# lslrh/DynaMask

Hardware: AMD Instinct MI355X
Metric: img/s (DynaMask mask-head path, 512 RoIs/img, fixed 28x28 exit; ms_per_step = ms per RoI batch) (higher is better)
Workload: dtype f32

## Files before the change

### dynamask_amd/csrc/deform_conv.hip

```cpp
#include "common.h"

namespace {

struct DcnArgs {
  const float* x;
  const float* offset;
  int NB, C, H, W, HW, Q;
  const float* wp;
  int Cout, CoutP, KQ, dg, relu;
  int q_begin = 0;
  float* out;
  int MT;
  float* ws = nullptr;
  long long ws_stride = 0, ws_floats = 0;
  int ksplit = 1, kchan = 0;
  const float* w2t = nullptr;
  const float* b2 = nullptr;
  float* out2 = nullptr;
  int M2 = 0, w2_ld = 0, out2_ct = 0, store_out = 1;
};

typedef float dm_f32x2 __attribute__((ext_vector_type(2)));

__device__ __forceinline__ float dcn_bilinear(float wt0, float wt1, float wb0, float wb1, float ta, float tb, float ba, float bb) {
  return __builtin_fmaf(wb1, bb, __builtin_fmaf(wb0, ba, __builtin_fmaf(wt1, tb, wt0 * ta)));
}

template <int WGM, int WGN, int WM, int WN>
__global__ __launch_bounds__(WGM* WGN * 64) void deform_conv_kernel(DcnArgs a) {
  constexpr int CK = 8;
  constexpr int TM = WGM * WM * 32;
  constexpr int TN = WGN * WN * 32;
  constexpr int NT = WGM * WGN * 64;
  constexpr int TG = NT / TN;
  constexpr int MAXT = (9 + TG - 1) / TG;
  constexpr int A_F4 = 9 * 2 * TM;
  constexpr int A_PER_T = (A_F4 + NT - 1) / NT;
  static_assert(NT % TN == 0, "threads must tile the pixel columns");

  extern __shared__ __attribute__((aligned(16))) float lds[];
  const int kc_begin = (a.ksplit > 1) ? (int)blockIdx.y * a.kchan : 0;
  const int kc_end = (a.ksplit > 1) ? min(a.C, kc_begin + a.kchan) : a.C;
  float* const e_out = (a.ksplit > 1) ? a.ws + (size_t)blockIdx.y * a.ws_stride : a.out;
  const int e_relu = (a.ksplit > 1) ? 0 : a.relu;
  dm_f32x4* ldsA = reinterpret_cast<dm_f32x4*>(lds);
  dm_f32x4* ldsB = reinterpret_cast<dm_f32x4*>(lds) + A_F4;

  const int tid = threadIdx.x;
  const int lane = tid & 63, wave = tid >> 6;
  const int wave_m = wave / WGN, wave_n = wave % WGN;
  const int hi = lane >> 5, l31 = lane & 31;
  int m_tile, n_tile;
  {
    const int b = blockIdx.x, grp = 8 * a.MT;
    const int full = (gridDim.x / grp) * grp;
    if (b < full) {
      const int g = b / grp, r = b - g * grp;
      m_tile = r / 8;
      n_tile = g * 8 + (r & 7);
    } else {
      const int r = b - full;
      m_tile = r % a.MT;
      n_tile = full / a.MT + r / a.MT;
    }
  }
  const int m0 = m_tile * TM;
  const int q0 = a.q_begin + n_tile * TN;
  const int HW = a.HW, W = a.W, H = a.H;

  int col_n[WN], col_p[WN];
  bool col_ok[WN];
#pragma unroll
  for (int wn = 0; wn < WN; ++wn) {
    int q = q0 + (wave_n * WN + wn) * 32 + l31;
    col_ok[wn] = q < a.Q;
    q = min(q, a.Q - 1);
    col_n[wn] = q / HW;
    col_p[wn] = q - col_n[wn] * HW;
  }

  const int gj = tid % TN;
  const int tg = tid / TN;
  int gq = q0 + gj;
  const bool g_ok = gq < a.Q;
  gq = min(gq, a.Q - 1);
  const int gn = gq / HW;
  const int gp = gq - gn * HW;
  const int gy = gp / W, gx = gp - gy * W;

  int ot[MAXT], ob[MAXT];
  float wt0[MAXT], wt1[MAXT], wb0[MAXT], wb1[MAXT];
  int cur_group = -1;
  const int cpg = a.C / a.dg;

  auto load_params = [&](int group) {
    const float* offp = a.offset + ((size_t)gn * a.dg + group) * 18 * HW + gp;
#pragma unroll
    for (int t = 0; t < MAXT; ++t) {
      const int tap = tg + t * TG;
      ot[t] = ob[t] = 0;
      wt0[t] = wt1[t] = wb0[t] = wb1[t] = 0.f;
      if (tap < 9 && g_ok) {
        const int ki = tap / 3, kj = tap - ki * 3;
        const float off_h = offp[(size_t)(2 * tap) * HW];
        const float off_w = offp[(size_t)(2 * tap + 1) * HW];
        const float h_im = (float)(gy - 1 + ki) + off_h;
        const float w_im = (float)(gx - 1 + kj) + off_w;
        if (h_im > -1.f && w_im > -1.f && h_im < (float)H && w_im < (float)W) {
          const int h_low = (int)floorf(h_im), w_low = (int)floorf(w_im);
          const float lh = h_im - (float)h_low, lw = w_im - (float)w_low;
          const float hh = 1.f - lh, hw = 1.f - lw;
          const float wr_t = (h_low >= 0) ? hh : 0.f;
          const float wr_b = (h_low + 1 <= H - 1) ? lh : 0.f;
          const int rt = min(max(h_low, 0), H - 1), rbm = min(max(h_low + 1, 0), H - 1);
          const int cb = min(max(w_low, 0), W - 2);
          const float wc0 = (cb == w_low ? hw : 0.f) + (cb == w_low + 1 ? lw : 0.f);
          const float wc1 = (cb + 1 == w_low ? hw : 0.f) + (cb + 1 == w_low + 1 ? lw : 0.f);
          ot[t] = rt * W + cb;
          ob[t] = rbm * W + cb;
          wt0[t] = wr_t * wc0; wt1[t] = wr_t * wc1;
          wb0[t] = wr_b * wc0; wb1[t] = wr_b * wc1;
        }
      }
    }
  };

  dm_f32x16 acc[WM][WN];
#pragma unroll
  for (int i = 0; i < WM; ++i)
#pragma unroll
    for (int j = 0; j < WN; ++j)
#pragma unroll
      for (int r = 0; r < 16; ++r) acc[i][j][r] = 0.f;

  struct __attribute__((packed, aligned(4))) F2 { float a, b; };
  dm_f32x4 ra[A_PER_T];
  dm_f32x4 raw[MAXT * 4];
  dm_f32x4 rb0[MAXT];

  auto prefetch_a = [&](int c0) {
#pragma unroll
    for (int i = 0; i < A_PER_T; ++i) {
      const int idx = tid + i * NT;
      dm_f32x4 v = {0.f, 0.f, 0.f, 0.f};
      if (idx < A_F4) {
        const int m = idx % TM;
        const int tq = idx / TM;
        const int qd = tq & 1;
        const int tap = tq >> 1;
        if (m0 + m < a.CoutP)
          v = *reinterpret_cast<const dm_f32x4*>(a.wp + (((size_t)tap * a.KQ + (c0 >> 2) + qd) * a.CoutP + m0 + m) * 4);
      }
      ra[i] = v;
    }
  };
  auto issue_quad = [&](int c0, int qd) {
    const float* xp = a.x + ((size_t)gn * a.C + c0 + qd * 4) * HW;
#pragma unroll
    for (int t = 0; t < MAXT; ++t) {
#pragma unroll
      for (int e = 0; e < 4; ++e) {
        const float* xc = xp + (size_t)e * HW;
        const F2 top = *reinterpret_cast<const F2*>(xc + ot[t]);
        const F2 bot = *reinterpret_cast<const F2*>(xc + ob[t]);
        dm_f32x4 v = {top.a, top.b, bot.a, bot.b};
        raw[t * 4 + e] = v;
      }
    }
  };
  auto combine = [&](int t) {
    dm_f32x4 v;
#pragma unroll
    for (int e = 0; e < 4; ++e) {
      const dm_f32x4 l = raw[t * 4 + e];
      v[e] = dcn_bilinear(wt0[t], wt1[t], wb0[t], wb1[t], l[0], l[1], l[2], l[3]);
// ... 211 lines not shown
    for (int i = 0; i < A_PER_T; ++i) {
      const int idx = tid + i * NT;
      const int m = idx % TM, tq = idx / TM;
      const int mm = min(m0 + m, a.CoutP - 1);
      ra[i] = *reinterpret_cast<const dm_f32x4*>(a.wp + (((size_t)(3 * g + (tq >> 1)) * a.KQ + (c0 >> 2) + (tq & 1)) * a.CoutP + mm) * 4);
    }
  };
  auto store_a = [&](int slot) {
#pragma unroll
    for (int i = 0; i < A_PER_T; ++i) ldsA[slot * AS_F4 + tid + i * NT] = ra[i];
  };
  auto load_x = [&](int c0) {
    const float* xc = a.x + ((size_t)n0 * a.C + c0) * HW;
#pragma unroll
    for (int i = 0; i < X_PER_T; ++i) {
#pragma unroll
      for (int e = 0; e < 4; ++e) rx[i][e] = xc[x_off[i] + e * HW];
    }
  };
  auto store_x = [&](int buf) {
#pragma unroll
    for (int i = 0; i < X_PER_T; ++i) {
      const int idx = tid + i * NT;
      if (idx < 4 * HW) ldsX[buf * xbuf + idx] = rx[i];
    }
  };
  auto gather3 = [&](int t0, int slot, int buf) {
    const dm_f32x4* xq = ldsX + buf * xbuf + xbase;
#pragma unroll
    for (int u = 0; u < 3; ++u) {
      const int tap = t0 + u;
      const dm_f32x4* pt = xq + (otb[tap] & 0xffff);
      const dm_f32x4* pb = xq + (otb[tap] >> 16);
      const dm_f32x4 tl = pt[0], tr = pt[1], bl = pb[0], br = pb[1];
      dm_f32x4 v;
#pragma unroll
      for (int e = 0; e < 4; ++e) v[e] = dcn_bilinear(wt0[tap], wt1[tap], wb0[tap], wb1[tap], tl[e], tr[e], bl[e], br[e]);
      ldsB[slot * BS_F4 + (u * 2 + gh) * TN + gj] = v;
    }
  };
  auto step = [&](int slot, bool fill, int t0, int gbuf) {
    const dm_f32x4* xq = ldsX + gbuf * xbuf + xbase;
#pragma unroll
    for (int u = 0; u < 3; ++u) {
      dm_f32x4 av[2], bv[2];
#pragma unroll
      for (int i = 0; i < 2; ++i) av[i] = ldsA[slot * AS_F4 + (u * 2 + hi) * TM + (wave_m * 2 + i) * 32 + l31];
#pragma unroll
      for (int j = 0; j < 2; ++j) bv[j] = ldsB[slot * BS_F4 + (u * 2 + hi) * TN + (wave_n * 2 + j) * 32 + l31];
      const int tap = t0 + u;
      dm_f32x4 tl, tr, bl, br;
      if (fill) {
        const dm_f32x4* pt = xq + (otb[tap] & 0xffff);
        const dm_f32x4* pb = xq + (otb[tap] >> 16);
        tl = pt[0]; tr = pt[1]; bl = pb[0]; br = pb[1];
      }
      __builtin_amdgcn_sched_barrier(0);
#pragma unroll
      for (int e = 0; e < 2; ++e)
#pragma unroll
        for (int i = 0; i < 2; ++i)
#pragma unroll
          for (int j = 0; j < 2; ++j) acc[i][j] = __builtin_amdgcn_mfma_f32_32x32x2f32(av[i][e], bv[j][e], acc[i][j], 0, 0, 0);
      __builtin_amdgcn_sched_barrier(0);
      if (fill) {
        dm_f32x4 v;
#pragma unroll
        for (int e = 0; e < 4; ++e) v[e] = dcn_bilinear(wt0[tap], wt1[tap], wb0[tap], wb1[tap], tl[e], tr[e], bl[e], br[e]);
        ldsB[(slot ^ 1) * BS_F4 + (u * 2 + gh) * TN + gj] = v;
      }
      __builtin_amdgcn_sched_barrier(0);
#pragma unroll
      for (int e = 2; e < 4; ++e)
#pragma unroll
        for (int i = 0; i < 2; ++i)
#pragma unroll
          for (int j = 0; j < 2; ++j) acc[i][j] = __builtin_amdgcn_mfma_f32_32x32x2f32(av[i][e], bv[j][e], acc[i][j], 0, 0, 0);
      __builtin_amdgcn_sched_barrier(0);
    }
  };

  int cur_group = kc_begin / cpg;
  load_params(cur_group);
  load_x(kc_begin);
  load_a(kc_begin, 0);
  store_x(0);
  store_a(0);
  load_a(kc_begin, 1);
  __syncthreads();
  gather3(0, 0, 0);
  __syncthreads();
  int slot = 0;
  for (int c0 = kc_begin, buf = 0; c0 < kc_end; c0 += 8, buf ^= 1) {
    const int cn = c0 + 8;
    const bool more = cn < kc_end;
    if (more) load_x(cn);
    store_a(slot ^ 1);
    load_a(c0, 2);
    step(slot, true, 3, buf);
    __syncthreads();
    slot ^= 1;
    store_a(slot ^ 1);
    if (more) {
      load_a(cn, 0);
      store_x(buf ^ 1);
    }
    step(slot, true, 6, buf);
    __syncthreads();
    slot ^= 1;
    if (more) {
      const int group = cn / cpg;
      if (group != cur_group) {
        cur_group = group;
        load_params(group);
      }
      store_a(slot ^ 1);
      load_a(cn, 1);
    }
    step(slot, more, 0, buf ^ 1);
    __syncthreads();
    slot ^= 1;
  }

  {
    float* pj[2];
#pragma unroll
    for (int j = 0; j < 2; ++j) pj[j] = e_out + (size_t)col_n[j] * a.Cout * HW + col_p[j];
    const int co_lane = m0 + wave_m * 64 + 4 * hi;
    const size_t off_lane = (size_t)co_lane * HW;
    const bool relu = e_relu != 0;
#pragma unroll
    for (int i = 0; i < 2; ++i)
#pragma unroll
      for (int r = 0; r < 16; ++r) {
        const int k = i * 32 + (r & 3) + 8 * (r >> 2);
        if (co_lane + k < a.Cout) {
          const size_t o = off_lane + (size_t)k * HW;
#pragma unroll
          for (int j = 0; j < 2; ++j)
            if (col_ok[j]) {
              float v = acc[i][j][r];
              if (relu) v = fmaxf(v, 0.f);
              pj[j][o] = v;
            }
        }
      }
  }
}

__global__ __launch_bounds__(256, 2) void deform_conv_c256_kernel(DcnArgs a) {
  constexpr int TN = 64, NT = 256;
  constexpr int BS_F4 = 3 * 2 * TN;
  constexpr int X_PER_T = 4;
  extern __shared__ __attribute__((aligned(16))) float lds[];
  dm_f32x4* ldsB = reinterpret_cast<dm_f32x4*>(lds);
  dm_f32x4* ldsX = ldsB + 2 * BS_F4;

  const int tid = threadIdx.x, lane = tid & 63, wave = tid >> 6;
  const int hi = lane >> 5, l31 = lane & 31;
  const int q0 = a.q_begin + (int)blockIdx.x * TN;
  const int HW = a.HW, W = a.W, H = a.H;
  const int n0 = q0 / HW;
  const int xbuf = 2 * 2 * HW;

  const int gj = tid & 63, gh = (tid >> 6) & 1, rb = tid >> 7;
  int gq = q0 + gj;
  const bool g_ok = gq < a.Q;
  gq = min(gq, a.Q - 1);
  const int gn = gq / HW, gp = gq - gn * HW;
  const int gy = gp / W, gx = gp - gy * W;
  const int xbase = ((gn - n0) * 2 + gh) * HW;

  int otb[3][2];
  float wt0[3][2], wt1[3][2], wb0[3][2], wb1[3][2];
  const int cpg = a.C / a.dg;
  auto load_params = [&](int group) {
    const float* offp = a.offset + ((size_t)gn * a.dg + group) * 18 * HW + gp;
#pragma unroll
    for (int s = 0; s < 3; ++s)
#pragma unroll
      for (int r = 0; r < 2; ++r) {
        otb[s][r] = 0;
        wt0[s][r] = wt1[s][r] = wb0[s][r] = wb1[s][r] = 0.f;
        if (g_ok) {
          const int ki = s, kj = r ? 2 : rb, tap = 3 * s + kj;
          const float h_im = (float)(gy - 1 + ki) + offp[(size_t)(2 * tap) * HW];
          const float w_im = (float)(gx - 1 + kj) + offp[(size_t)(2 * tap + 1) * HW];
          if (h_im > -1.f && w_im > -1.f && h_im < (float)H && w_im < (float)W) {
            const int h_low = (int)floorf(h_im), w_low = (int)floorf(w_im);
            const float lh = h_im - (float)h_low, lw = w_im - (float)w_low;
            const float hh = 1.f - lh, hw = 1.f - lw;
            const float wr_t = (h_low >= 0) ? hh : 0.f;
            const float wr_b = (h_low + 1 <= H - 1) ? lh : 0.f;
            const int rt = min(max(h_low, 0), H - 1), rbm = min(max(h_low + 1, 0), H - 1);
            const int cb = min(max(w_low, 0), W - 2);
            const float wc0 = (cb == w_low ? hw : 0.f) + (cb == w_low + 1 ? lw : 0.f);
            const float wc1 = (cb + 1 == w_low ? hw : 0.f) + (cb + 1 == w_low + 1 ? lw : 0.f);
            otb[s][r] = (rt * W + cb) | ((rbm * W + cb) << 16);
            wt0[s][r] = wr_t * wc0; wt1[s][r] = wr_t * wc1;
            wb0[s][r] = wr_b * wc0; wb1[s][r] = wr_b * wc1;
          }
        }
      }
  };

  dm_f32x16 acc[2][2];
#pragma unroll
  for (int i = 0; i < 2; ++i)
#pragma unroll
    for (int j = 0; j < 2; ++j)
#pragma unroll
      for (int r = 0; r < 16; ++r) acc[i][j][r] = 0.f;

  dm_f32x4 rx[X_PER_T];
  const __amdgpu_buffer_rsrc_t xsrc = __builtin_amdgcn_make_buffer_rsrc(
      const_cast<float*>(a.x) + (size_t)n0 * a.C * HW, 0, min(2, a.NB - n0) * a.C * HW * 4, 0x00020000);
  const __amdgpu_buffer_rsrc_t wsrc = __builtin_amdgcn_make_buffer_rsrc(const_cast<float*>(a.wp), 0, 9 * a.KQ * a.CoutP * 16, 0x00020000);
  unsigned x_off[X_PER_T];
#pragma unroll
  for (int i = 0; i < X_PER_T; ++i) {
    const int idx = tid + i * NT;
    const int img = idx / (2 * HW), r = idx - img * 2 * HW;
    const int quad = r / HW, px = r - quad * HW;
    const int ii = (idx < 4 * HW) ? img : 0, qq = (idx < 4 * HW) ? quad : 0, pp = (idx < 4 * HW) ? px : 0;
    x_off[i] = 4u * (unsigned)(((min(n0 + ii, a.NB - 1) - n0) * a.C + qq * 4) * HW + pp);
  }
  unsigned a_off[2];
#pragma unroll
  for (int i = 0; i < 2; ++i) a_off[i] = 16u * (unsigned)(hi * a.CoutP + min(wave * 64 + i * 32 + l31, a.CoutP - 1));
  const int a_quad = a.CoutP * 16, a_tap = a.KQ * a_quad;
  auto load_a1 = [&](dm_f32x4 (&dst)[6], int c0, int g, int u) {
    const int so = (3 * g + u) * a_tap + (c0 >> 2) * a_quad;
#pragma unroll
    for (int i = 0; i < 2; ++i) dst[u * 2 + i] = __builtin_bit_cast(dm_f32x4, __builtin_amdgcn_raw_buffer_load_b128(wsrc, a_off[i], so, 0));
  };
  auto load_x = [&](int c0) {
#pragma unroll
    for (int e = 0; e < 4; ++e) {
      const int so = (c0 + e) * HW * 4;
#pragma unroll
      for (int i = 0; i < X_PER_T; ++i) rx[i][e] = __builtin_bit_cast(float, __builtin_amdgcn_raw_buffer_load_b32(xsrc, x_off[i], so, 0));
    }
  };
  auto store_x = [&](int buf) {
#pragma unroll
    for (int i = 0; i < X_PER_T; ++i) {
      const int idx = tid + i * NT;
      if (idx < 4 * HW) ldsX[buf * xbuf + idx] = rx[i];
    }
  };
  auto whole_read = [&](const dm_f32x4* xq, int s, dm_f32x4& tl, dm_f32x4& tr, dm_f32x4& bl, dm_f32x4& br) {
    const dm_f32x4* pt = xq + (otb[s][0] & 0xffff);
    const dm_f32x4* pb = xq + (otb[s][0] >> 16);
    tl = pt[0]; tr = pt[1]; bl = pb[0]; br = pb[1];
  };
  auto whole_write = [&](int slot, int s, const dm_f32x4& tl, const dm_f32x4& tr, const dm_f32x4& bl, const dm_f32x4& br) {
    dm_f32x4 v;
#pragma unroll
    for (int e = 0; e < 4; ++e) v[e] = dcn_bilinear(wt0[s][0], wt1[s][0], wb0[s][0], wb1[s][0], tl[e], tr[e], bl[e], br[e]);
    ldsB[slot * BS_F4 + (rb * 2 + gh) * TN + gj] = v;
  };
  auto half_read = [&](const dm_f32x4* xq, int s, dm_f32x2& tl, dm_f32x2& tr, dm_f32x2& bl, dm_f32x2& br) {
    const dm_f32x2* pt = reinterpret_cast<const dm_f32x2*>(xq + (otb[s][1] & 0xffff)) + rb;
    const dm_f32x2* pb = reinterpret_cast<const dm_f32x2*>(xq + (otb[s][1] >> 16)) + rb;
    tl = pt[0]; tr = pt[2]; bl = pb[0]; br = pb[2];
  };
  auto half_write = [&](int slot, int s, const dm_f32x2& tl, const dm_f32x2& tr, const dm_f32x2& bl, const dm_f32x2& br) {
    dm_f32x2 v;
#pragma unroll
    for (int e = 0; e < 2; ++e) v[e] = dcn_bilinear(wt0[s][1], wt1[s][1], wb0[s][1], wb1[s][1], tl[e], tr[e], bl[e], br[e]);
    reinterpret_cast<dm_f32x2*>(&ldsB[slot * BS_F4 + (2 * 2 + gh) * TN + gj])[rb] = v;
  };
  auto step = [&](const dm_f32x4 (&cur)[6], dm_f32x4 (&nxt)[6], int slot, bool fill, int sn, int gbuf, bool pre, int pc0, int pg) {
    const dm_f32x4* xq = ldsX + gbuf * xbuf + xbase;
#pragma unroll
    for (int u = 0; u < 3; ++u) {
      dm_f32x4 bv[2];
#pragma unroll
      for (int j = 0; j < 2; ++j) bv[j] = ldsB[slot * BS_F4 + (u * 2 + hi) * TN + j * 32 + l31];
      dm_f32x4 tl, tr, bl, br;
      dm_f32x2 htl, htr, hbl, hbr;
      if (fill && u == 0) whole_read(xq, sn, tl, tr, bl, br);
      if (fill && u == 1) half_read(xq, sn, htl, htr, hbl, hbr);
      if (pre) load_a1(nxt, pc0, pg, u);
      __builtin_amdgcn_sched_barrier(0);
#pragma unroll
      for (int e = 0; e < 2; ++e)
#pragma unroll
        for (int i = 0; i < 2; ++i)
#pragma unroll
          for (int j = 0; j < 2; ++j) acc[i][j] = __builtin_amdgcn_mfma_f32_32x32x2f32(cur[u * 2 + i][e], bv[j][e], acc[i][j], 0, 0, 0);
      __builtin_amdgcn_sched_barrier(0);
      if (fill && u == 0) whole_write(slot ^ 1, sn, tl, tr, bl, br);
      if (fill && u == 1) half_write(slot ^ 1, sn, htl, htr, hbl, hbr);
      __builtin_amdgcn_sched_barrier(0);
#pragma unroll
      for (int e = 2; e < 4; ++e)
#pragma unroll
        for (int i = 0; i < 2; ++i)
#pragma unroll
          for (int j = 0; j < 2; ++j) acc[i][j] = __builtin_amdgcn_mfma_f32_32x32x2f32(cur[u * 2 + i][e], bv[j][e], acc[i][j], 0, 0, 0);
      __builtin_amdgcn_sched_barrier(0);
    }
  };
  int cur_group = 0;
  auto chunk = [&](dm_f32x4 (&p)[6], dm_f32x4 (&q)[6], int c0, int buf, int slot) {
    const int cn = c0 + 8;
    const bool more = cn < a.C;
    if (more) load_x(cn);
    step(p, q, slot, true, 1, buf, true, c0, 1);
    __syncthreads();
    if (more) store_x(buf ^ 1);
    step(q, p, slot ^ 1, true, 2, buf, true, c0, 2);
    __syncthreads();
    if (more) {
      const int group = cn / cpg;
      if (group != cur_group) {
        cur_group = group;
        load_params(group);
      }
    }
    step(p, q, slot, more, 0, buf ^ 1, more, cn, 0);
    __syncthreads();
  };

  dm_f32x4 a0[6], a1[6];
  load_params(0);
  load_x(0);
#pragma unroll
  for (int u = 0; u < 3; ++u) load_a1(a0, 0, 0, u);
  store_x(0);
  __syncthreads();
  {
    const dm_f32x4* xq = ldsX + xbase;
    dm_f32x4 tl, tr, bl, br;
    dm_f32x2 htl, htr, hbl, hbr;
    whole_read(xq, 0, tl, tr, bl, br);
    half_read(xq, 0, htl, htr, hbl, hbr);
    whole_write(0, 0, tl, tr, bl, br);
    half_write(0, 0, htl, htr, hbl, hbr);
  }
  __syncthreads();
  for (int c0 = 0; c0 < a.C; c0 += 16) {
    chunk(a0, a1, c0, 0, 0);
    if (c0 + 8 < a.C) chunk(a1, a0, c0 + 8, 1, 1);
  }

  {
    float* pj[2];
    bool col_ok[2];
#pragma unroll
    for (int j = 0; j < 2; ++j) {
      int q = q0 + j * 32 + l31;
      col_ok[j] = q < a.Q;
      q = min(q, a.Q - 1);
      const int n = q / HW;
      pj[j] = a.out + (size_t)n * a.Cout * HW + (q - n * HW);
    }
    const int co_lane = wave * 64 + 4 * hi;
    const size_t off_lane = (size_t)co_lane * HW;
    const bool relu = a.relu != 0;
#pragma unroll
    for (int i = 0; i < 2; ++i)
#pragma unroll
      for (int r = 0; r < 16; ++r) {
        const int k = i * 32 + (r & 3) + 8 * (r >> 2);
        if (co_lane + k < a.Cout) {
          const size_t o = off_lane + (size_t)k * HW;
#pragma unroll
          for (int j = 0; j < 2; ++j)
            if (col_ok[j]) {
              float v = acc[i][j][r];
              if (relu) v = fmaxf(v, 0.f);
              pj[j][o] = v;
            }
        }
      }
  }
}

constexpr int DCN_NEAR_ROWS = 5;

template <int WM, int WGM, int XR>
__global__ __launch_bounds__(256, 2) void deform_conv_band_kernel(DcnArgs a, int tiles_per_img, int BR) {
  constexpr int TM = WM * WGM * 32, TN = (4 / WGM) * 32, NT = 256;
  constexpr int A_F4 = 9 * 2 * TM;
  constexpr int A_PER_T = (A_F4 + NT - 1) / NT;
  extern __shared__ __attribute__((aligned(16))) float lds[];
  const int kc_begin = (a.ksplit > 1) ? (int)blockIdx.y * a.kchan : 0;
  const int kc_end = (a.ksplit > 1) ? min(a.C, kc_begin + a.kchan) : a.C;
  float* const e_out = (a.ksplit > 1) ? a.ws + (size_t)blockIdx.y * a.ws_stride : a.out;
  const int e_relu = (a.ksplit > 1) ? 0 : a.relu;
  dm_f32x4* ldsA = reinterpret_cast<dm_f32x4*>(lds);
  dm_f32x4* ldsX = reinterpret_cast<dm_f32x4*>(lds) + A_F4;
  const int tid = threadIdx.x, lane = tid & 63, wave = tid >> 6;
  const int hi = lane >> 5, l31 = lane & 31;
  const int wave_m = wave % WGM, wave_n = wave / WGM;
  const int HW = a.HW, W = a.W, H = a.H;
  const int PS = BR * W, PS4 = PS >> 2;
  const int n = blockIdx.x / tiles_per_img, tile = blockIdx.x - n * tiles_per_img;
  const int p0 = tile * TN;
  const int p_end = min(p0 + TN, HW);
  const int y_first = p0 / W, y_last = (p_end - 1) / W;
  const int band_y0 = min(max(y_first - (BR - (y_last - y_first + 1)) / 2, 0), H - BR);
  int gp = p0 + wave_n * 32 + l31;
  const bool g_ok = gp < HW;
  gp = min(gp, HW - 1);
  const int gy = gp / W, gx = gp - gy * W;

  int otb[9];
  float wt0[9], wt1[9], wb0[9], wb1[9];
  unsigned oob = 0, any_oob = 0;
  const int cpg = a.C / a.dg;
  auto load_params = [&](int group) {
    const float* offp = a.offset + ((size_t)n * a.dg + group) * 18 * HW + gp;
    oob = 0;
#pragma unroll
    for (int tap = 0; tap < 9; ++tap) {
      otb[tap] = 0;
      wt0[tap] = wt1[tap] = wb0[tap] = wb1[tap] = 0.f;
      if (g_ok) {
        const int ki = tap / 3, kj = tap - ki * 3;
        const float h_im = (float)(gy - 1 + ki) + offp[(size_t)(2 * tap) * HW];
        const float w_im = (float)(gx - 1 + kj) + offp[(size_t)(2 * tap + 1) * HW];
        if (h_im > -1.f && w_im > -1.f && h_im < (float)H && w_im < (float)W) {
          const int h_low = (int)floorf(h_im), w_low = (int)floorf(w_im);
          const float lh = h_im - (float)h_low, lw = w_im - (float)w_low;
          const float hh = 1.f - lh, hw = 1.f - lw;
          const float wr_t = (h_low >= 0) ? hh : 0.f;
          const float wr_b = (h_low + 1 <= H - 1) ? lh : 0.f;
          const int rt = min(max(h_low, 0), H - 1), rbm = min(max(h_low + 1, 0), H - 1);
          const int cb = min(max(w_low, 0), W - 2);
          const float wc0 = (cb == w_low ? hw : 0.f) + (cb == w_low + 1 ? lw : 0.f);
          const float wc1 = (cb + 1 == w_low ? hw : 0.f) + (cb + 1 == w_low + 1 ? lw : 0.f);
          if (rt >= gy - DCN_NEAR_ROWS && rbm <= gy + DCN_NEAR_ROWS) {
            otb[tap] = ((rt - band_y0) * W + cb) | (((rbm - band_y0) * W + cb) << 16);
            wt0[tap] = wr_t * wc0; wt1[tap] = wr_t * wc1;
            wb0[tap] = wr_b * wc0; wb1[tap] = wr_b * wc1;
          } else {
            oob |= 1u << tap;
          }
        }
      }
    }
    any_oob = 0;
#pragma unroll
    for (int tap = 0; tap < 9; ++tap)
      if (__ballot((oob >> tap) & 1u) != 0ull) any_oob |= 1u << tap;
  };

  dm_f32x16 acc[WM];
#pragma unroll
  for (int i = 0; i < WM; ++i)
#pragma unroll
    for (int r = 0; r < 16; ++r) acc[i][r] = 0.f;

  dm_f32x4 ra[A_PER_T], rx[XR];
  unsigned a_off[A_PER_T];
#pragma unroll
  for (int i = 0; i < A_PER_T; ++i) {
    const int idx = min(tid + i * NT, A_F4 - 1);
    const int m = idx % TM, tq = idx / TM;
    a_off[i] = (unsigned)((((size_t)(tq >> 1) * a.KQ + (tq & 1)) * a.CoutP + min(m, a.CoutP - 1)) * 4);
  }
  auto load_a = [&](int c0) {
    const float* wb = a.wp + (size_t)(c0 >> 2) * a.CoutP * 4;
#pragma unroll
    for (int i = 0; i < A_PER_T; ++i) ra[i] = *reinterpret_cast<const dm_f32x4*>(wb + a_off[i]);
  };
  auto load_x = [&](int c0) {
    const float* xb = a.x + ((size_t)n * a.C + c0) * HW + (size_t)band_y0 * W;
#pragma unroll
    for (int i = 0; i < XR; ++i) {
      const int idx = tid + i * NT;
      const int off = (idx < PS) ? idx : (idx < 2 * PS ? 4 * HW + idx - PS : 0);
#pragma unroll
      for (int e = 0; e < 4; ++e) rx[i][e] = xb[off + e * HW];
    }
  };
  auto store_ax = [&]() {
#pragma unroll
    for (int i = 0; i < A_PER_T; ++i) {
      const int idx = tid + i * NT;
      if (idx < A_F4) ldsA[idx] = ra[i];
    }
#pragma unroll
    for (int i = 0; i < XR; ++i) {
      const int idx = tid + i * NT;
      if (idx < 2 * PS) ldsX[idx] = rx[i];
    }
  };
  struct __attribute__((packed, aligned(4))) F2 { float a, b; };

  int cur_group = kc_begin / cpg;
  load_params(cur_group);
  load_a(kc_begin);
  load_x(kc_begin);
  for (int c0 = kc_begin; c0 < kc_end; c0 += 8) {
// ... 95 lines not shown
    {
      const dm_f32x4* src = reinterpret_cast<const dm_f32x4*>(a.w2t);
      dm_f32x4* dst = reinterpret_cast<dm_f32x4*>(lds);
      for (int idx = tid; idx < a.Cout * (ld2 / 4); idx += NT) dst[idx] = src[idx];
    }
    __syncthreads();
    const float* w2t = lds;
    dm_f32x16 acc2[MT2];
#pragma unroll
    for (int t = 0; t < MT2; ++t)
#pragma unroll
      for (int r = 0; r < 16; ++r) acc2[t][r] = 0.f;
#pragma unroll
    for (int i = 0; i < WM; ++i)
#pragma unroll
      for (int r = 0; r < 16; ++r) {
        const int kb = i * 32 + (r & 3) + 8 * (r >> 2) + 4 * hi;
        const float b = fmaxf(acc[i][r], 0.f);
#pragma unroll
        for (int t = 0; t < MT2; ++t)
          if (t * 32 < ld2) acc2[t] = __builtin_amdgcn_mfma_f32_32x32x2f32(w2t[kb * ld2 + t * 32 + l31], b, acc2[t], 0, 0, 0);
      }
    const int p = p0 + wave_n * 32 + l31;
    if (p < HW) {
      float* po2 = a.out2 + (size_t)n * a.out2_ct * HW + p;
#pragma unroll
      for (int t = 0; t < MT2; ++t)
#pragma unroll
        for (int r = 0; r < 16; ++r) {
          const int co = t * 32 + (r & 3) + 8 * (r >> 2) + 4 * hi;
          if (co < a.M2) po2[(size_t)co * HW] = fmaxf(acc2[t][r] + a.b2[co], 0.f);
        }
    }
    if (!a.store_out) return;
  }
  {
    const int p = p0 + wave_n * 32 + l31;
    if (p < HW) {
      float* po = e_out + (size_t)n * a.Cout * HW + p;
      const bool relu = e_relu != 0;
#pragma unroll
      for (int i = 0; i < WM; ++i)
#pragma unroll
        for (int r = 0; r < 16; ++r) {
          const int co = (wave_m * WM + i) * 32 + (r & 3) + 8 * (r >> 2) + 4 * hi;
          if (co < a.Cout) {
            float v = acc[i][r];
            if (relu) v = fmaxf(v, 0.f);
            po[(size_t)co * HW] = v;
          }
        }
    }
  }
}

__global__ __launch_bounds__(256) void dcn_splitk_reduce_kernel(const float* __restrict__ ws, int splits, long long stride,
                                                               long long total, int relu, float* __restrict__ out) {
  const bool v4 = splits > 0;
  splits = v4 ? splits : -splits;
  if (v4) {
    const float4* ws4 = reinterpret_cast<const float4*>(ws);
    float4* out4 = reinterpret_cast<float4*>(out);
    const long long total4 = total >> 2, stride4 = stride >> 2;
    for (long long e = (long long)blockIdx.x * blockDim.x + threadIdx.x; e < total4; e += (long long)gridDim.x * blockDim.x) {
      float4 v = ws4[e];
      for (int s_ = 1; s_ < splits; ++s_) {
        const float4 w = ws4[(size_t)s_ * stride4 + e];
        v.x += w.x; v.y += w.y; v.z += w.z; v.w += w.w;
      }
      if (relu) { v.x = fmaxf(v.x, 0.f); v.y = fmaxf(v.y, 0.f); v.z = fmaxf(v.z, 0.f); v.w = fmaxf(v.w, 0.f); }
      out4[e] = v;
    }
    return;
  }
  for (long long e = (long long)blockIdx.x * blockDim.x + threadIdx.x; e < total; e += (long long)gridDim.x * blockDim.x) {
    float v = ws[e];
    for (int s_ = 1; s_ < splits; ++s_) v += ws[(size_t)s_ * stride + e];
    out[e] = relu ? fmaxf(v, 0.f) : v;
  }
}

static void dcn_choose_split(DcnArgs& a, long long wgs, long long slots, long long ws_floats, bool lds_tiles = false) {
  a.ksplit = 1;
  if (!a.ws || a.q_begin != 0 || wgs <= 0) return;
  const int chunks = a.C / 8;
  const long long per = (long long)a.NB * a.Cout * a.HW;
  int S = 1;
  if (a.NB <= 24) {
    long long Smax = min(min(8LL, slots / wgs), (long long)chunks / 2);
    if (per > 0) Smax = min(Smax, ws_floats / per);
    const double chain_us = chunks * 3.5, out_mb = (double)per * 4e-6;
    double best = 8.0;
    for (int c = 2; c <= Smax; ++c) {
      const double g = chain_us * (1.0 - 1.0 / c) - (5.0 + (c + 1) * out_mb * 0.25);
      if (g > best) { best = g; S = c; }
    }
  } else if (lds_tiles && wgs < slots && chunks >= 12 && per > 0 && ws_floats / per >= 3) {
    S = 3;
  }
  if (S >= 2) {
    const int per_split = dm_ceil_div(chunks, S);
    a.kchan = per_split * 8;
    a.ksplit = dm_ceil_div(chunks, per_split);
    a.ws_stride = per;
  }
}

static int dcn_finish_split(const DcnArgs& a, int relu, float* out, hipStream_t st) {
  if (a.ksplit <= 1) return dm_check_launch();
  int rc = dm_check_launch();
  if (rc != DM_OK) return rc;
  const long long total = a.ws_stride;
  const bool v4 = (total & 3) == 0 && ((((uintptr_t)a.ws) | ((uintptr_t)out)) & 15) == 0;
  DM_LAUNCH(dcn_splitk_reduce_kernel, dim3((unsigned)min((long long)4096, ((v4 ? total / 4 : total) + 255) / 256)), dim3(256), 0, st, a.ws,
            v4 ? a.ksplit : -a.ksplit, a.ws_stride, total, relu, out);
  return dm_check_launch();
}

template <int WM, int WGM, int XR>
int launch_dcn_band(DcnArgs& a, hipStream_t st) {
  const int BR = 16;
  if (8 * BR * a.W / 4 > XR * 256 || a.H < BR) return DM_ERR_UNSUPPORTED;
  const int tiles = dm_ceil_div(a.HW, (4 / WGM) * 32);
  const size_t lds_bytes = 16 * (size_t)(9 * 2 * WM * WGM * 32) + 4 * (size_t)8 * BR * a.W;
  if (a.w2t) {
    if (WGM != 1 || a.w2_ld != dm_ceil_div(a.M2, 32) * 32 || a.w2_ld > (WM + 1) / 2 * 32 || (size_t)a.Cout * a.w2_ld * 4 > lds_bytes ||
        a.Cout != WM * 32)
      return DM_ERR_UNSUPPORTED;
    a.ws = nullptr;
  }
  dcn_choose_split(a, (long long)a.NB * tiles, 2LL * dm_num_cus(), a.ws_floats);
  DM_LAUNCH((deform_conv_band_kernel<WM, WGM, XR>), dim3((unsigned)(a.NB * tiles), (unsigned)a.ksplit), dim3(256), lds_bytes, st, a, tiles, BR);
  return dcn_finish_split(a, a.relu, a.out, st);
}

template <int WGM, int WGN, int WM, int WN>
int launch_dcn(DcnArgs& a, hipStream_t st) {
  constexpr int TM = WGM * WM * 32;
  constexpr int TN = WGN * WN * 32;
  constexpr int NT = WGM * WGN * 64;
  a.MT = dm_ceil_div(a.CoutP, TM);
  const int NTiles = dm_ceil_div(a.Q - a.q_begin, TN);
  const size_t lds_bytes = 16 * ((size_t)9 * 2 * TM + (size_t)2 * 9 * TN);
  static bool attr_set[DM_MAX_DEVICES] = {false};
  if (lds_bytes > 64 * 1024 &&
      dm_ensure_lds_limit(reinterpret_cast<const void*>(&deform_conv_kernel<WGM, WGN, WM, WN>), (int)lds_bytes, attr_set) != DM_OK)
    return DM_ERR_LAUNCH;
  dcn_choose_split(a, (long long)a.MT * NTiles, (NT == 256 ? 2LL : 1LL) * dm_num_cus(), a.ws_floats);
  DM_LAUNCH((deform_conv_kernel<WGM, WGN, WM, WN>), dim3(a.MT * NTiles, a.ksplit), dim3(NT), lds_bytes, st, a);
  return dcn_finish_split(a, a.relu, a.out, st);
}

int launch_dcn_c256(DcnArgs& a, bool tail, hipStream_t st) {
  const size_t lds_bytes = 16 * ((size_t)2 * 3 * 2 * 64) + (size_t)4 * 2 * 2 * 8 * a.HW;
  const int NTiles = dm_ceil_div(a.Q, 64);
  const int slots = 2 * dm_num_cus();
  const int full_rounds = NTiles / slots;
  const int rem = NTiles - full_rounds * slots;
  a.ksplit = 1;
  if (tail && full_rounds >= 1 && rem > 0 && rem * 20 <= 3 * slots) {
    const int n_main = full_rounds * slots;
    const int Q = a.Q;
    a.Q = n_main * 64;
    DM_LAUNCH(deform_conv_c256_kernel, dim3(n_main), dim3(256), lds_bytes, st, a);
    int rc = dm_check_launch();
    if (rc != DM_OK) return rc;
    a.q_begin = a.Q;
    a.Q = Q;
    return launch_dcn<2, 2, 1, 1>(a, st);
  }
  DM_LAUNCH(deform_conv_c256_kernel, dim3(NTiles), dim3(256), lds_bytes, st, a);
  return dm_check_launch();
}

}

struct DcnTout {
  const float* w2t = nullptr;
  const float* b2 = nullptr;
  float* out2 = nullptr;
  int M2 = 0, out2_ct = 0;
};
static int deform_conv_fwd_impl(const float* x, const float* offset, int NB, int C, int H, int W,
                                const float* w_packed, int Cout, int deform_groups, int relu, float* out, float* ws,
                                long long ws_floats, dm_stream_t stream, const DcnTout* tout = nullptr);

extern "C" int dm_deform_conv_fwd(const float* x, const float* offset, int NB, int C, int H, int W,
                                  const float* w_packed, int Cout, int deform_groups, int relu, float* out,
                                  dm_stream_t stream) {
  return deform_conv_fwd_impl(x, offset, NB, C, H, W, w_packed, Cout, deform_groups, relu, out, nullptr, 0, stream);
}

extern "C" long long dm_deform_conv_splitk_floats(int NB, int C, int H, int W, int Cout) {
  if (NB <= 0 || C < 32 || H <= 0 || W <= 0 || Cout <= 0) return 0;
  const long long wgs = (long long)dm_ceil_div(Cout, 128) * dm_ceil_div((long long)NB * H * W, 128);
  if (wgs * 2 > 2LL * dm_num_cus() && !(H * W <= 256 && wgs < 2LL * dm_num_cus())) return 0;
  return 8LL * NB * Cout * H * W;
}

extern "C" int dm_deform_conv_fwd_ws(const float* x, const float* offset, int NB, int C, int H, int W,
                                     const float* w_packed, int Cout, int deform_groups, int relu, float* out,
                                     float* workspace, long long workspace_floats, dm_stream_t stream) {
  return deform_conv_fwd_impl(x, offset, NB, C, H, W, w_packed, Cout, deform_groups, relu, out, workspace, workspace_floats, stream);
}

static bool dcn_tout_shape_ok(int NB, int C, int H, int W, int Cout, int M2) {
  if (NB <= 0 || C <= 0 || H <= 0 || W <= 0 || Cout != C || M2 <= 0) return false;
  const int HW = H * W, CoutP = dm_conv_packed_cout(Cout);
  const int max_rows = (W - 1 + 128 + W - 1) / W;
  if (!(H >= 16 && (W & 3) == 0 && 8 * 16 * W / 4 <= 7 * 256 && (16 - max_rows) / 2 >= DCN_NEAR_ROWS && HW > 256 && HW < 65536 &&
        (CoutP == 64 || CoutP == 128) && Cout > 32 && Cout == CoutP))
    return false;
  const bool narrow = 8 * 16 * W / 4 <= 4 * 256;
  const bool few = (long long)NB * dm_ceil_div(HW, 128) * 4 < (long long)dm_num_cus() * 3;
  if (few) return false;
  if (CoutP == 128 && !narrow) return false;
  return dm_ceil_div(M2, 32) <= (CoutP / 32 + 1) / 2;
}

extern "C" int dm_deform_conv_tout_supported(int NB, int C, int H, int W, int Cout, int M2) {
  return dcn_tout_shape_ok(NB, C, H, W, Cout, M2) ? 1 : 0;
}

extern "C" int dm_deform_conv_tout_fwd(const float* x, const float* offset, int NB, int C, int H, int W, const float* w_packed,
                                       int Cout, int deform_groups, const float* w2t, const float* b2, int M2, float* out2,
                                       int out2_ch_total, float* out_dcn, dm_stream_t stream) {
  if (!w2t || !b2 || !out2 || M2 <= 0 || M2 > out2_ch_total) return DM_ERR_INVALID_ARG;
  if (NB == 0) return DM_OK;
  if (!dcn_tout_shape_ok(NB, C, H, W, Cout, M2)) return DM_ERR_UNSUPPORTED;
  DcnTout t;
  t.w2t = w2t; t.b2 = b2; t.out2 = out2; t.M2 = M2; t.out2_ct = out2_ch_total;
  return deform_conv_fwd_impl(x, offset, NB, C, H, W, w_packed, Cout, deform_groups, 1, out_dcn ? out_dcn : out2, nullptr, 0, stream,
                              &t) ;
}

static int deform_conv_fwd_impl(const float* x, const float* offset, int NB, int C, int H, int W,
                                const float* w_packed, int Cout, int deform_groups, int relu, float* out, float* ws,
                                long long ws_floats, dm_stream_t stream, const DcnTout* tout) {
  if (!x || !offset || !w_packed || !out) return DM_ERR_INVALID_ARG;
  if (relu & 16) return DM_ERR_UNSUPPORTED;
  if (NB < 0 || C <= 0 || H <= 0 || W <= 0 || Cout <= 0 || deform_groups <= 0 || C % deform_groups != 0)
    return DM_ERR_INVALID_ARG;
  if ((long long)NB * H * W > 0x7fffffffLL) return DM_ERR_INVALID_ARG;
  if ((C / deform_groups) % 8 != 0) return DM_ERR_UNSUPPORTED;
  if (W < 2) return DM_ERR_UNSUPPORTED;
  if (NB == 0) return DM_OK;
  DcnArgs a;
  a.x = x; a.offset = offset; a.NB = NB; a.C = C; a.H = H; a.W = W; a.HW = H * W; a.Q = NB * H * W;
  a.wp = w_packed; a.Cout = Cout; a.CoutP = dm_conv_packed_cout(Cout); a.KQ = (C + 7) / 8 * 2; a.dg = deform_groups;
  a.relu = relu & 1; a.out = out;
  a.ws = (ws && ws_floats > 0) ? ws : nullptr;
  a.ws_floats = a.ws ? ws_floats : 0;
  if (tout) {
    a.w2t = tout->w2t; a.b2 = tout->b2; a.out2 = tout->out2; a.M2 = tout->M2; a.w2_ld = dm_ceil_div(tout->M2, 32) * 32;
    a.out2_ct = tout->out2_ct;
    a.store_out = (out != tout->out2) ? 1 : 0;
  }
  hipStream_t st = (hipStream_t)stream;
  {
    const int max_rows = (W - 1 + 128 + W - 1) / W;
    if (H >= 16 && (W & 3) == 0 && 8 * 16 * W / 4 <= 7 * 256 && (16 - max_rows) / 2 >= DCN_NEAR_ROWS && a.HW > 256 &&
        a.HW < 65536 && (a.CoutP == 64 || a.CoutP == 128) && Cout > 32) {
      const bool narrow = 8 * 16 * W / 4 <= 4 * 256;
      bool few = (long long)NB * dm_ceil_div(a.HW, 128) * 4 < (long long)dm_num_cus() * 3;
      if (few && a.ws && NB <= 24 && !tout) few = false;
      if (a.CoutP == 64) {
        if (few) return narrow ? launch_dcn_band<1, 2, 4>(a, st) : launch_dcn_band<1, 2, 7>(a, st);
        return narrow ? launch_dcn_band<2, 1, 4>(a, st) : launch_dcn_band<2, 1, 7>(a, st);
      }
      if (few) return narrow ? launch_dcn_band<1, 4, 4>(a, st) : launch_dcn_band<1, 4, 7>(a, st);
      return narrow ? launch_dcn_band<4, 1, 4>(a, st) : launch_dcn_band<2, 2, 7>(a, st);
    }
  }
  if (tout) return DM_ERR_UNSUPPORTED;
  const bool lds_split = a.ws && Cout > 64 && a.HW >= 128 && a.HW <= 256 && (a.HW & 3) == 0;
  if (!lds_split && Cout > 64 &&
      (long long)dm_ceil_div(a.CoutP, 128) * dm_ceil_div(a.Q, 128) * 20 <= (long long)dm_num_cus() * 9)
    return launch_dcn<2, 2, 1, 1>(a, st);
  if (Cout > 64 && a.HW >= 128 && a.HW <= 256 && (a.HW & 3) == 0 && (C / deform_groups) % 8 == 0) {
    a.MT = dm_ceil_div(a.CoutP, 128);
    const int NTiles = dm_ceil_div(a.Q, 128);
    const size_t lds_bytes = 16 * ((size_t)2 * 2 * 3 * 2 * 128) + (size_t)4 * 2 * 2 * 8 * a.HW;
    static bool attr_lds[DM_MAX_DEVICES] = {false};
    if (dm_ensure_lds_limit(reinterpret_cast<const void*>(&deform_conv_lds_kernel), 16 * 2 * 2 * 3 * 2 * 128 + 4 * 2 * 2 * 8 * 256,
                            attr_lds) != DM_OK)
      return DM_ERR_LAUNCH;
    static const int tail_mode = getenv("DM_DCN_TAIL") ? atoi(getenv("DM_DCN_TAIL")) : 1;
    const int slots = 2 * dm_num_cus();
    if (a.CoutP == 256) {
      dcn_choose_split(a, (long long)a.MT * NTiles, slots, a.ws_floats, true);
      if (a.ksplit == 1) return launch_dcn_c256(a, tail_mode && !(relu & 8), st);
    }
    const int full_rounds = (a.MT * NTiles) / slots;
    const int rem = a.MT * NTiles - full_rounds * slots;
    if (tail_mode && !(relu & 8) && full_rounds >= 1 && rem > 0 && rem * 20 <= 3 * slots) {
      const int n_main = full_rounds * slots / a.MT;
      const int Q = a.Q;
      a.Q = n_main * 128;
      DM_LAUNCH(deform_conv_lds_kernel, dim3(a.MT * n_main), dim3(256), lds_bytes, st, a);
      int rc = dm_check_launch();
      if (rc != DM_OK) return rc;
      a.q_begin = a.Q;
      a.Q = Q;
      return launch_dcn<2, 2, 1, 1>(a, st);
    }
    dcn_choose_split(a, (long long)a.MT * NTiles, slots, a.ws_floats, true);
    DM_LAUNCH(deform_conv_lds_kernel, dim3(a.MT * NTiles, a.ksplit), dim3(256), lds_bytes, st, a);
// ... 9 lines not shown
```

Measured before the change: 298.5.

## Prefetch DCN offsets via buffer loads and specialise chunk loop at compile time

Reworks the c256 deformable-conv kernel's main loop. Offset values are now prefetched through buffer loads one stage ahead of when the bilinear parameters are computed, instead of being loaded and consumed synchronously at a group boundary. The parameter computation is made branchless. The last chunk is peeled so the feed and prefetch flags become compile-time template flags, and the weight offset goes through readfirstlane. The LDS x-buffer is sized to a fixed 4*NT slots, and the bounds check on the store is dropped. This risks reading past 4*HW if the spatial size changes, and adds register pressure from holding the prefetched offsets.

```diff
diff --git a/dynamask_amd/csrc/deform_conv.hip b/dynamask_amd/csrc/deform_conv.hip
--- a/dynamask_amd/csrc/deform_conv.hip
+++ b/dynamask_amd/csrc/deform_conv.hip
@@ -21,6 +21,11 @@
 };
 
 typedef float dm_f32x2 __attribute__((ext_vector_type(2)));
+
+template <bool B>
+struct dcn_flag {
+  static constexpr bool value = B;
+};
 
 __device__ __forceinline__ float dcn_bilinear(float wt0, float wt1, float wb0, float wb1, float ta, float tb, float ba, float bb) {
   return __builtin_fmaf(wb1, bb, __builtin_fmaf(wb0, ba, __builtin_fmaf(wt1, tb, wt0 * ta)));
@@ -538,6 +543,7 @@
   constexpr int TN = 64, NT = 256;
   constexpr int BS_F4 = 3 * 2 * TN;
   constexpr int X_PER_T = 4;
+  constexpr int XBUF = X_PER_T * NT;
   extern __shared__ __attribute__((aligned(16))) float lds[];
   dm_f32x4* ldsB = reinterpret_cast<dm_f32x4*>(lds);
   dm_f32x4* ldsX = ldsB + 2 * BS_F4;
@@ -547,7 +553,6 @@
   const int q0 = a.q_begin + (int)blockIdx.x * TN;
   const int HW = a.HW, W = a.W, H = a.H;
   const int n0 = q0 / HW;
-  const int xbuf = 2 * 2 * HW;
 
   const int gj = tid & 63, gh = (tid >> 6) & 1, rb = tid >> 7;
   int gq = q0 + gj;
@@ -559,34 +564,28 @@
 
   int otb[3][2];
   float wt0[3][2], wt1[3][2], wb0[3][2], wb1[3][2];
-  const int cpg = a.C / a.dg;
-  auto load_params = [&](int group) {
-    const float* offp = a.offset + ((size_t)gn * a.dg + group) * 18 * HW + gp;
+  auto set_params = [&](const float (&po)[12]) {
 #pragma unroll
     for (int s = 0; s < 3; ++s)
 #pragma unroll
       for (int r = 0; r < 2; ++r) {
-        otb[s][r] = 0;
-        wt0[s][r] = wt1[s][r] = wb0[s][r] = wb1[s][r] = 0.f;
-        if (g_ok) {
-          const int ki = s, kj = r ? 2 : rb, tap = 3 * s + kj;
-          const float h_im = (float)(gy - 1 + ki) + offp[(size_t)(2 * tap) * HW];
-          const float w_im = (float)(gx - 1 + kj) + offp[(size_t)(2 * tap + 1) * HW];
-          if (h_im > -1.f && w_im > -1.f && h_im < (float)H && w_im < (float)W) {
-            const int h_low = (int)floorf(h_im), w_low = (int)floorf(w_im);
-            const float lh = h_im - (float)h_low, lw = w_im - (float)w_low;
-            const float hh = 1.f - lh, hw = 1.f - lw;
-            const float wr_t = (h_low >= 0) ? hh : 0.f;
-            const float wr_b = (h_low + 1 <= H - 1) ? lh : 0.f;
-            const int rt = min(max(h_low, 0), H - 1), rbm = min(max(h_low + 1, 0), H - 1);
-            const int cb = min(max(w_low, 0), W - 2);
-            const float wc0 = (cb == w_low ? hw : 0.f) + (cb == w_low + 1 ? lw : 0.f);
-            const float wc1 = (cb + 1 == w_low ? hw : 0.f) + (cb + 1 == w_low + 1 ? lw : 0.f);
-            otb[s][r] = (rt * W + cb) | ((rbm * W + cb) << 16);
-            wt0[s][r] = wr_t * wc0; wt1[s][r] = wr_t * wc1;
-            wb0[s][r] = wr_b * wc0; wb1[s][r] = wr_b * wc1;
-          }
-        }
+        const int ki = s, kj = r ? 2 : rb;
+        const float h_off = (float)(gy - 1 + ki) + po[2 * (2 * s + r)];
+        const float w_off = (float)(gx - 1 + kj) + po[2 * (2 * s + r) + 1];
+        const bool in = g_ok && h_off > -1.f && w_off > -1.f && h_off < (float)H && w_off < (float)W;
+        const float h_im = in ? h_off : 0.f, w_im = in ? w_off : 0.f;
+        const int h_low = (int)floorf(h_im), w_low = (int)floorf(w_im);
+        const float lh = h_im - (float)h_low, lw = w_im - (float)w_low;
+        const float hh = 1.f - lh, hw = 1.f - lw;
+        const float wr_t = (h_low >= 0) ? hh : 0.f;
+        const float wr_b = (h_low + 1 <= H - 1) ? lh : 0.f;
+        const int rt = min(max(h_low, 0), H - 1), rbm = min(max(h_low + 1, 0), H - 1);
+        const int cb = min(max(w_low, 0), W - 2);
+        const float wc0 = (cb == w_low ? hw : 0.f) + (cb == w_low + 1 ? lw : 0.f);
+        const float wc1 = (cb + 1 == w_low ? hw : 0.f) + (cb + 1 == w_low + 1 ? lw : 0.f);
+        otb[s][r] = in ? (rt * W + cb) | ((rbm * W + cb) << 16) : 0;
+        wt0[s][r] = in ? wr_t * wc0 : 0.f; wt1[s][r] = in ? wr_t * wc1 : 0.f;
+        wb0[s][r] = in ? wr_b * wc0 : 0.f; wb1[s][r] = in ? wr_b * wc1 : 0.f;
       }
   };
 
@@ -602,6 +601,21 @@
   const __amdgpu_buffer_rsrc_t xsrc = __builtin_amdgcn_make_buffer_rsrc(
       const_cast<float*>(a.x) + (size_t)n0 * a.C * HW, 0, min(2, a.NB - n0) * a.C * HW * 4, 0x00020000);
   const __amdgpu_buffer_rsrc_t wsrc = __builtin_amdgcn_make_buffer_rsrc(const_cast<float*>(a.wp), 0, 9 * a.KQ * a.CoutP * 16, 0x00020000);
+  const __amdgpu_buffer_rsrc_t osrc = __builtin_amdgcn_make_buffer_rsrc(
+      const_cast<float*>(a.offset) + (size_t)n0 * a.dg * 18 * HW, 0, min(2, a.NB - n0) * a.dg * 18 * HW * 4, 0x00020000);
+  const unsigned o_half = 4u * (unsigned)((gn - n0) * a.dg * 18 * HW + gp);
+  const unsigned o_whole = o_half + 4u * (unsigned)(2 * rb * HW);
+  auto load_offs = [&](float (&po)[12], int group) {
+#pragma unroll
+    for (int s = 0; s < 3; ++s)
+#pragma unroll
+      for (int r = 0; r < 2; ++r)
+#pragma unroll
+        for (int d = 0; d < 2; ++d) {
+          const int so = ((group * 18 + 2 * (3 * s + (r ? 2 : 0)) + d) * HW) * 4;
+          po[2 * (2 * s + r) + d] = __builtin_bit_cast(float, __builtin_amdgcn_raw_buffer_load_b32(osrc, r ? o_half : o_whole, so, 0));
+        }
+  };
   unsigned x_off[X_PER_T];
 #pragma unroll
   for (int i = 0; i < X_PER_T; ++i) {
@@ -616,7 +630,7 @@
   for (int i = 0; i < 2; ++i) a_off[i] = 16u * (unsigned)(hi * a.CoutP + min(wave * 64 + i * 32 + l31, a.CoutP - 1));
   const int a_quad = a.CoutP * 16, a_tap = a.KQ * a_quad;
   auto load_a1 = [&](dm_f32x4 (&dst)[6], int c0, int g, int u) {
-    const int so = (3 * g + u) * a_tap + (c0 >> 2) * a_quad;
+    const int so = __builtin_amdgcn_readfirstlane((3 * g + u) * a_tap + (c0 >> 2) * a_quad);
 #pragma unroll
     for (int i = 0; i < 2; ++i) dst[u * 2 + i] = __builtin_bit_cast(dm_f32x4, __builtin_amdgcn_raw_buffer_load_b128(wsrc, a_off[i], so, 0));
   };
@@ -630,10 +644,7 @@
   };
   auto store_x = [&](int buf) {
 #pragma unroll
-    for (int i = 0; i < X_PER_T; ++i) {
-      const int idx = tid + i * NT;
-      if (idx < 4 * HW) ldsX[buf * xbuf + idx] = rx[i];
-    }
+    for (int i = 0; i < X_PER_T; ++i) ldsX[buf * XBUF + tid + i * NT] = rx[i];
   };
   auto whole_read = [&](const dm_f32x4* xq, int s, dm_f32x4& tl, dm_f32x4& tr, dm_f32x4& bl, dm_f32x4& br) {
     const dm_f32x4* pt = xq + (otb[s][0] & 0xffff);
@@ -657,8 +668,9 @@
     for (int e = 0; e < 2; ++e) v[e] = dcn_bilinear(wt0[s][1], wt1[s][1], wb0[s][1], wb1[s][1], tl[e], tr[e], bl[e], br[e]);
     reinterpret_cast<dm_f32x2*>(&ldsB[slot * BS_F4 + (2 * 2 + gh) * TN + gj])[rb] = v;
   };
-  auto step = [&](const dm_f32x4 (&cur)[6], dm_f32x4 (&nxt)[6], int slot, bool fill, int sn, int gbuf, bool pre, int pc0, int pg) {
-    const dm_f32x4* xq = ldsX + gbuf * xbuf + xbase;
+  auto step = [&](auto feed_flag, const dm_f32x4 (&cur)[6], dm_f32x4 (&nxt)[6], int slot, int sn, int gbuf, int pc0, int pg) {
+    constexpr bool feed = decltype(feed_flag)::value;
+    const dm_f32x4* xq = ldsX + gbuf * XBUF + xbase;
 #pragma unroll
     for (int u = 0; u < 3; ++u) {
       dm_f32x4 bv[2];
@@ -666,9 +678,11 @@
       for (int j = 0; j < 2; ++j) bv[j] = ldsB[slot * BS_F4 + (u * 2 + hi) * TN + j * 32 + l31];
       dm_f32x4 tl, tr, bl, br;
       dm_f32x2 htl, htr, hbl, hbr;
-      if (fill && u == 0) whole_read(xq, sn, tl, tr, bl, br);
-      if (fill && u == 1) half_read(xq, sn, htl, htr, hbl, hbr);
-      if (pre) load_a1(nxt, pc0, pg, u);
+      if constexpr (feed) {
+        if (u == 0) whole_read(xq, sn, tl, tr, bl, br);
+        if (u == 1) half_read(xq, sn, htl, htr, hbl, hbr);
+        load_a1(nxt, pc0, pg, u);
+      }
       __builtin_amdgcn_sched_barrier(0);
 #pragma unroll
       for (int e = 0; e < 2; ++e)
@@ -677,8 +691,10 @@
 #pragma unroll
           for (int j = 0; j < 2; ++j) acc[i][j] = __builtin_amdgcn_mfma_f32_32x32x2f32(cur[u * 2 + i][e], bv[j][e], acc[i][j], 0, 0, 0);
       __builtin_amdgcn_sched_barrier(0);
-      if (fill && u == 0) whole_write(slot ^ 1, sn, tl, tr, bl, br);
-      if (fill && u == 1) half_write(slot ^ 1, sn, htl, htr, hbl, hbr);
+      if constexpr (feed) {
+        if (u == 0) whole_write(slot ^ 1, sn, tl, tr, bl, br);
+        if (u == 1) half_write(slot ^ 1, sn, htl, htr, hbl, hbr);
+      }
       __builtin_amdgcn_sched_barrier(0);
 #pragma unroll
       for (int e = 2; e < 4; ++e)
@@ -689,32 +705,36 @@
       __builtin_amdgcn_sched_barrier(0);
     }
   };
-  int cur_group = 0;
-  auto chunk = [&](dm_f32x4 (&p)[6], dm_f32x4 (&q)[6], int c0, int buf, int slot) {
+  float po[12];
+  const int group_chunks = a.C / a.dg / 8;
+  int group = 0, group_left = group_chunks;
+  auto chunk = [&](auto more_flag, dm_f32x4 (&p)[6], dm_f32x4 (&q)[6], int c0, int buf, int slot) {
+    constexpr bool more = decltype(more_flag)::value;
     const int cn = c0 + 8;
-    const bool more = cn < a.C;
-    if (more) load_x(cn);
-    step(p, q, slot, true, 1, buf, true, c0, 1);
+    if constexpr (more) load_x(cn);
+    step(dcn_flag<true>{}, p, q, slot, 1, buf, c0, 1);
     __syncthreads();
-    if (more) store_x(buf ^ 1);
-    step(q, p, slot ^ 1, true, 2, buf, true, c0, 2);
+    bool turn = false;
+    if constexpr (more) {
+      store_x(buf ^ 1);
+      turn = group_left == 1;
+      group_left = turn ? group_chunks : group_left - 1;
+      if (turn) load_offs(po, ++group);
+    }
+    step(dcn_flag<true>{}, q, p, slot ^ 1, 2, buf, c0, 2);
     __syncthreads();
-    if (more) {
-      const int group = cn / cpg;
-      if (group != cur_group) {
-        cur_group = group;
-        load_params(group);
-      }
-    }
-    step(p, q, slot, more, 0, buf ^ 1, more, cn, 0);
+    if (turn) set_params(po);
+    step(more_flag, p, q, slot, 0, buf ^ 1, cn, 0);
     __syncthreads();
   };
 
   dm_f32x4 a0[6], a1[6];
-  load_params(0);
+  load_offs(po, 0);
   load_x(0);
 #pragma unroll
   for (int u = 0; u < 3; ++u) load_a1(a0, 0, 0, u);
+  __builtin_amdgcn_sched_barrier(0);
+  set_params(po);
   store_x(0);
   __syncthreads();
   {
@@ -727,9 +747,20 @@
     half_write(0, 0, htl, htr, hbl, hbr);
   }
   __syncthreads();
-  for (int c0 = 0; c0 < a.C; c0 += 16) {
-    chunk(a0, a1, c0, 0, 0);
-    if (c0 + 8 < a.C) chunk(a1, a0, c0 + 8, 1, 1);
+  {
+    int c0 = 0, par = 0;
+    for (; c0 + 16 < a.C; c0 += 16) {
+      chunk(dcn_flag<true>{}, a0, a1, c0, 0, 0);
+      chunk(dcn_flag<true>{}, a1, a0, c0 + 8, 1, 1);
+    }
+    if (c0 + 8 < a.C) {
+      chunk(dcn_flag<true>{}, a0, a1, c0, 0, 0);
+#pragma unroll
+      for (int k = 0; k < 6; ++k) a0[k] = a1[k];
+      par = 1;
+      c0 += 8;
+    }
+    chunk(dcn_flag<false>{}, a0, a1, c0, par, par);
   }
 
   {
@@ -1131,7 +1162,7 @@
 }
 
 int launch_dcn_c256(DcnArgs& a, bool tail, hipStream_t st) {
-  const size_t lds_bytes = 16 * ((size_t)2 * 3 * 2 * 64) + (size_t)4 * 2 * 2 * 8 * a.HW;
+  const size_t lds_bytes = 16 * ((size_t)2 * 3 * 2 * 64) + (size_t)16 * 2 * 4 * 256;
   const int NTiles = dm_ceil_div(a.Q, 64);
   const int slots = 2 * dm_num_cus();
   const int full_rounds = NTiles / slots;
```

Result: no change. 300.0 (median of 6 runs) (+0.5%).
